# TheoBald200814/RGB-D-Instance-Segmentation

Hardware: AMD Instinct MI355X
Metric: NYUv2 640x480 RGB-D img/s (fwd+bwd) of the DGGM+E-DSAM hot path (higher is better)
Workload: dtype bf16

## Files before the change

### include/rgbd_hip.h

```cpp
#ifndef RGBD_HIP_H
#define RGBD_HIP_H

#include <stddef.h>
#include <stdint.h>

#ifdef __cplusplus
extern "C" {
#endif

#define RGBD_OK 0
#define RGBD_E_ARG (-1)
#define RGBD_E_SHAPE (-2)
#define RGBD_E_DTYPE (-3)

#define RGBD_F32 0
#define RGBD_BF16 1

#define RGBD_NBINS 512
#define RGBD_MAX_MODES 3

typedef struct rgbd_decomp_info {
  int32_t status;
  int32_t n_modes;
  int32_t n_masks;
// ... 64 lines not shown
                             const int* C_host, const int* h_host, const int* w_host, const float* grad,
                             const float* mask, long long pv_batch_stride, int B, int H, int W, void* ws,
                             void* stream);

int rgbd_nchw_to_nhwc(int dtype, const void* src, void* dst, int B, int C, int H, int W,
                      void* stream);
typedef struct rgbd_nhwc_job {
  const void* src;
  void* dst;
  int B, C, H, W;
} rgbd_nhwc_job;
int rgbd_nchw_to_nhwc_multi(int n, const rgbd_nhwc_job* jobs, void* stream);
typedef struct rgbd_nhwc_job_f32 {
  const void* src;
  void* dst;
  int B, C, H, W;
  int dst_dtype;
} rgbd_nhwc_job_f32;
int rgbd_nchw_to_nhwc_multi_f32(int n, const rgbd_nhwc_job_f32* jobs, void* stream);
long long rgbd_dsam_packed_elems(int dtype, int Cin, int Cout);
int rgbd_dsam_pack_weights(int dtype, const float* conv_w, const float* proj_w, int Cin,
                           int Cout, const uint32_t* code_mask, void* wfwd, void* wbwd, void* stream);
int rgbd_dsam_code_masks(int n, const uint8_t* const* codes_host, const long long* nbytes_host,
                         uint32_t* masks, void* stream);

size_t rgbd_dsam_conv_workspace_size(int dtype, int B, int Cin, int h, int w, int Cout);
int rgbd_dsam_fwd(int dtype, const void* x_nhwc, const uint8_t* code, const rgbd_decomp_info* info,
                  int B, int Cin, int h, int w, int Cout, const void* wfwd, const float* bias,
                  const void* residual, void* out_nchw, void* out_nhwc, void* ws, void* stream);
int rgbd_dsam_fwd_nhwc(int dtype, const void* x_nhwc, const uint8_t* code, const rgbd_decomp_info* info,
                       int B, int Cin, int h, int w, int Cout, const void* wfwd, const float* bias,
                       const void* residual_nhwc, void* out_nhwc, void* ws, void* stream);
int rgbd_dsam_fwd_nhwc_f32io(int dtype, const void* x_nhwc, const uint8_t* code, const rgbd_decomp_info* info,
                             int B, int Cin, int h, int w, int Cout, const void* wfwd, const float* bias,
                             const void* residual_nhwc, void* out_nhwc, void* ws, void* stream,
                             const float* residual_f32_nhwc, float* out_f32_nhwc);
int rgbd_dsam_bwd_data(int dtype, const void* gout_nhwc, const uint8_t* code, int B, int Cin, int h,
                       int w, int Cout, const void* wbwd, const void* gin_nchw, const void* gin_nhwc,
                       void* dx_nchw, void* dx_nhwc, void* ws, void* stream);
size_t rgbd_dsam_bwd_weight_workspace_size(int dtype, int B, int Cin, int h, int w, int Cout);
int rgbd_dsam_bwd_weight(int dtype, const void* gout_nchw, const void* gout_nhwc, const void* x_nhwc,
                         const uint8_t* code, const rgbd_decomp_info* info, int B, int Cin, int h,
                         int w, int Cout, float* dconv_w, float* dproj_w, float* dbias, void* ws,
                         void* stream);

enum { RGBD_LEG_FWD = 0, RGBD_LEG_DX = 1, RGBD_LEG_DW = 2 };
typedef struct rgbd_dsam_leg {
  int kind;
  const uint8_t* code;
  int B, Cin, h, w, Cout;
  void* plan;
} rgbd_dsam_leg;
size_t rgbd_dsam_plan_size(int kind, int B, int Cin, int h, int w, int Cout);
size_t rgbd_dsam_run_workspace_size(int kind, int B, int Cin, int h, int w, int Cout);
int rgbd_dsam_plan(int n, const rgbd_dsam_leg* legs, void* stream);
int rgbd_dsam_fwd_nhwc_planned(int dtype, const void* x_nhwc, const uint8_t* code,
                               const rgbd_decomp_info* info, int B, int Cin, int h, int w, int Cout,
                               const void* wfwd, const float* bias, const void* residual_nhwc,
                               void* out_nhwc, const void* plan, void* ws, void* stream);
int rgbd_dsam_fwd_nhwc_f32io_planned(int dtype, const void* x_nhwc, const uint8_t* code,
                                     const rgbd_decomp_info* info, int B, int Cin, int h, int w, int Cout,
                                     const void* wfwd, const float* bias, const void* residual_nhwc, void* out_nhwc,
                                     const void* plan, void* ws, void* stream, const float* residual_f32_nhwc,
                                     float* out_f32_nhwc);
int rgbd_dsam_bwd_data_planned(int dtype, const void* gout_nhwc, const uint8_t* code, int B, int Cin,
                               int h, int w, int Cout, const void* wbwd, const void* gin_nchw,
                               const void* gin_nhwc, void* dx_nchw, void* dx_nhwc, const void* plan,
                               void* ws, void* stream);
int rgbd_dsam_bwd_weight_planned(int dtype, const void* gout_nchw, const void* gout_nhwc,
                                 const void* x_nhwc, const uint8_t* code, const rgbd_decomp_info* info,
                                 int B, int Cin, int h, int w, int Cout, float* dconv_w, float* dproj_w,
                                 float* dbias, const void* plan, void* ws, void* stream);
typedef struct rgbd_dsam_dw_run {
  const void* gout_nhwc;
  const void* x_nhwc;
  const uint8_t* code;
  int B, Cin, h, w, Cout;
  float* dconv_w;
  float* dproj_w;
  float* dbias;
  const void* plan;
  void* ws;
} rgbd_dsam_dw_run;
int rgbd_dsam_bwd_weight_planned_multi(int n, const rgbd_dsam_dw_run* runs, const rgbd_decomp_info* info,
                                       void* stream);

int rgbd_adamw_multi(int n, float* const* params, const float* const* grads, float* const* exp_avg,
                     float* const* exp_avg_sq, const long long* numel, const float* step, double lr, double beta1,
                     double beta2, double eps, double weight_decay, void* stream);
int rgbd_adamw_multi_shadow(int n, float* const* params, const float* const* grads, float* const* exp_avg,
                            float* const* exp_avg_sq, void* const* shadows, const long long* numel,
                            const float* step, double lr, double beta1, double beta2, double eps,
                            double weight_decay, void* stream);

#define RGBD_RATIO_NW 24
#define RGBD_RATIO_NBN 6
size_t rgbd_ratio_packed_size(int dtype);
int rgbd_ratio_pack(int dtype, const float* const* weights_host, void* packed, void* stream);
size_t rgbd_ratio_workspace_size(int dtype, int B, int H, int W);
size_t rgbd_ratio_features_offset(int dtype, int B, int H, int W);
size_t rgbd_ratio_pooled_offset(int dtype, int B, int H, int W);
int rgbd_ratio_forward(int dtype, int training, float momentum, const float* depth3, long long batch_stride,
                       int B, int H, int W, const void* packed, float* const* bn_host, unsigned long long seed,
                       unsigned long long* seed_counter, float* ratio, void* ws, void* stream);
#define RGBD_RATIO_F_PHASE2 1
int rgbd_ratio_forward_ex(int dtype, int training, float momentum, const float* depth3, long long batch_stride,
// ... 116 lines not shown
```

### rgb-d-instance-segmentation_amd/_lib.py

```python
import ctypes
import os
from pathlib import Path

import numpy as np

LIB_PATH = Path(os.environ.get("RGBD_HIP_LIB", Path(__file__).resolve().parent / "librgbd_hip.so"))

RGBD_F32 = 0
RGBD_BF16 = 1
NBINS = 512

DECOMP_INFO_DTYPE = np.dtype([
    ("status", "<i4"), ("n_modes", "<i4"), ("n_masks", "<i4"), ("peak_bin", "<i4", 3),
    ("first_edge", "<f4"), ("last_edge", "<f4"), ("center", "<f4", 3),
    ("lo", "<f4", 3), ("hi", "<f4", 3), ("hist", "<i4", NBINS)])
assert DECOMP_INFO_DTYPE.itemsize == 2116

_P = ctypes.c_void_p
_I = ctypes.c_int
_LL = ctypes.c_longlong
_SZ = ctypes.c_size_t

SIGNATURES = {
    "rgbd_version": (ctypes.c_char_p, []),
    "rgbd_assemble_workspace_size": (_SZ, [_I]),
    "rgbd_assemble_pixel_values": (_I, [_P, _P, _I, _I, _I, _P, _P, _P]),
    "rgbd_instance_presence": (_I, [_P, _I, _I, _I, _P, _P]),
    "rgbd_instance_masks": (_I, [_P, _I, _I, _P, _P, _I, _P, _P]),
    "rgbd_pp_instance_workspace_size": (_SZ, [_I, _I]),
    "rgbd_pp_instance": (_I, [_P, _P, _I, _I, _I, _I, _I, _P, _P, ctypes.c_double, _P, _P, _P, _P, _P, _P]),
    "rgbd_pp_binary_maps": (_I, [_P, _I, _I, _I, _I, _I, _P, _P, _P]),
    "rgbd_pack_mask_bits": (_I, [_P, _I, _LL, _P, _P, _P]),
    "rgbd_mask_intersections": (_I, [_P, _I, _P, _I, _LL, _P, _P]),
    "rgbd_resize_workspace_size": (_SZ, [_I, _I, _I, _I, _I, _I]),
    "rgbd_resize_pil_bilinear": (_I, [_P, _I, _I, _I, _I, _I, _I, _P, _P, _P]),
    "rgbd_resize_pil_nearest": (_I, [_P, _I, _I, _I, _I, _I, _I, _P, _P, _P]),
    "rgbd_resize_cv2_linear": (_I, [_P, _I, _I, _I, _I, _I, _P, _P, _P]),
    "rgbd_edsam_decompose_workspace_size": (_SZ, [_I]),
    "rgbd_edsam_decompose": (_I, [_P, _LL, _I, _I, _I, _I, _P, _I, _P, _P, _P, _P, _P, _P]),
    "rgbd_edsam_decompose_masks": (_I, [_P, _LL, _I, _I, _I, _I, _P, _I, _P, _P, _P, _P, _P, _P, _P]),
    "rgbd_edsam_modes_workspace_size": (_SZ, [_I, _I, _I]),
    "rgbd_edsam_modes": (_I, [_P, _LL, _I, _I, _I, _I, _P, _P, _I, _P, _P]),
    "rgbd_edsam_codes": (_I, [_P, _I, _I, _I, _P, _I, _P, _P, _P, _P, _P, _P]),
    "rgbd_dggm_fuse_fwd": (_I, [_I, _P, _P, _P, _P, _LL, _I, _I, _I, _I, _I, _I, _P, _P, _P, _P]),
    "rgbd_dggm_fuse_bwd_workspace_size": (_SZ, [_I, _I, _I, _I]),
    "rgbd_dggm_fuse_bwd": (_I, [_I, _P, _P, _P, _LL, _I, _I, _I, _I, _I, _I, _P, _P, _P, _P, _P, _P]),
    "rgbd_dggm_fuse_fwd_multi": (_I, [_I, _I, _P, _P, _P, _P, _P, _P, _P, _P, _P, _P, _LL, _I, _I, _I, _P]),
    "rgbd_dggm_fuse_fwd_multi_mixed": (_I, [_I, _I, _P, _I, _P, _P, _P, _P, _P, _P, _P, _P, _P, _LL, _I, _I, _I,
                                            _P]),
    "rgbd_dggm_fuse_bwd_multi_workspace_size": (_SZ, [_I, _P, _P, _P, _I]),
    "rgbd_dggm_fuse_bwd_multi": (_I, [_I, _I, _P, _P, _P, _P, _P, _P, _P, _P, _P, _P, _LL, _I, _I, _I, _P, _P]),
    "rgbd_nchw_to_nhwc": (_I, [_I, _P, _P, _I, _I, _I, _I, _P]),
    "rgbd_nchw_to_nhwc_multi": (_I, [_I, _P, _P]),
    "rgbd_nchw_to_nhwc_multi_f32": (_I, [_I, _P, _P]),
    "rgbd_adamw_multi": (_I, [_I, _P, _P, _P, _P, _P, _P, ctypes.c_double, ctypes.c_double, ctypes.c_double,
                             ctypes.c_double, ctypes.c_double, _P]),
    "rgbd_adamw_multi_shadow": (_I, [_I, _P, _P, _P, _P, _P, _P, _P, ctypes.c_double, ctypes.c_double,
                                     ctypes.c_double, ctypes.c_double, ctypes.c_double, _P]),
    "rgbd_dsam_packed_elems": (_LL, [_I, _I, _I]),
    "rgbd_dsam_pack_weights": (_I, [_I, _P, _P, _I, _I, _P, _P, _P, _P]),
    "rgbd_dsam_code_masks": (_I, [_I, _P, _P, _P, _P]),
    "rgbd_dsam_conv_workspace_size": (_SZ, [_I, _I, _I, _I, _I, _I]),
    "rgbd_dsam_fwd": (_I, [_I, _P, _P, _P, _I, _I, _I, _I, _I, _P, _P, _P, _P, _P, _P, _P]),
    "rgbd_dsam_fwd_nhwc": (_I, [_I, _P, _P, _P, _I, _I, _I, _I, _I, _P, _P, _P, _P, _P, _P]),
    "rgbd_dsam_bwd_data": (_I, [_I, _P, _P, _I, _I, _I, _I, _I, _P, _P, _P, _P, _P, _P, _P]),
    "rgbd_dsam_bwd_weight_workspace_size": (_SZ, [_I, _I, _I, _I, _I, _I]),
    "rgbd_dsam_bwd_weight": (_I, [_I, _P, _P, _P, _P, _P, _I, _I, _I, _I, _I, _P, _P, _P, _P, _P]),
    "rgbd_dsam_plan_size": (_SZ, [_I, _I, _I, _I, _I, _I]),
    "rgbd_dsam_run_workspace_size": (_SZ, [_I, _I, _I, _I, _I, _I]),
    "rgbd_dsam_plan": (_I, [_I, _P, _P]),
    "rgbd_dsam_fwd_nhwc_planned": (_I, [_I, _P, _P, _P, _I, _I, _I, _I, _I, _P, _P, _P, _P, _P, _P, _P]),
    "rgbd_dsam_fwd_nhwc_f32io": (_I, [_I, _P, _P, _P, _I, _I, _I, _I, _I, _P, _P, _P, _P, _P, _P, _P, _P]),
    "rgbd_dsam_fwd_nhwc_f32io_planned": (_I, [_I, _P, _P, _P, _I, _I, _I, _I, _I, _P, _P, _P, _P, _P, _P, _P, _P,
                                              _P]),
    "rgbd_dsam_bwd_data_planned": (_I, [_I, _P, _P, _I, _I, _I, _I, _I, _P, _P, _P, _P, _P, _P, _P, _P]),
    "rgbd_dsam_bwd_weight_planned": (_I, [_I, _P, _P, _P, _P, _P, _I, _I, _I, _I, _I, _P, _P, _P, _P, _P, _P]),
    "rgbd_dsam_bwd_weight_planned_multi": (_I, [_I, _P, _P, _P]),
    "rgbd_point_sample": (_I, [_P, _I, _I, _I, _P, _I, _I, _P, _P]),
    "rgbd_point_sample_t": (_I, [_I, _P, _I, _I, _I, _P, _I, _I, _P, _P]),
    "rgbd_point_sample_sets": (_I, [_I, _P, _I, _I, _I, _P, _P, _I, _P, _P]),
    "rgbd_topk_rows_max_n": (_SZ, []),
    "rgbd_topk_rows": (_I, [_P, _I, _I, _I, _P, _P]),
    "rgbd_point_sample_bwd": (_I, [_P, _I, _I, _I, _P, _I, _I, _P, _P]),
    "rgbd_match_cost": (_I, [_P, _I, _I, _I, _P, _P, _P, _P, ctypes.c_float, ctypes.c_float, ctypes.c_float, _P, _P]),
    "rgbd_match_cost_probs": (_I, [_P, _I, _I, _I, _P, _P, _P, _I, _P, _P, ctypes.c_float, ctypes.c_float,
                                   ctypes.c_float, _P, _P]),
    "rgbd_point_losses": (_I, [_P, _P, _I, _I, _P, _P, _P, _P]),
    "rgbd_point_losses_bwd": (_I, [_P, _P, _I, _I, _P, _P, _P, _P, _P]),
    "rgbd_msda_fwd": (_I, [_I, _P, _I, _I, _P, _I, _I, _I, _I, _P, _P, _P, _P]),
    "rgbd_msda_bwd": (_I, [_I, _P, _I, _I, _P, _I, _I, _I, _I, _P, _P, _P, _P, _P, _P, _P]),
    "rgbd_level_memory_workspace_size": (_SZ, [_I, _I, _I]),
    "rgbd_level_memory_fwd": (_I, [_I, _P, _P, _I, _I, _I, _P, _P]),
    "rgbd_level_memory_bwd": (_I, [_I, _P, _I, _I, _I, _P, _P, _P, _P]),
    "rgbd_msda_locations": (_I, [_I, _P, _P, _P, _I, _I, _I, _I, _I, _P, _P]),
    "rgbd_msda_locations_bwd": (_I, [_I, _P, _P, _I, _I, _I, _I, _I, _P, _P]),
    "rgbd_lsa_lds_bytes": (_SZ, [_I, _I]),
    "rgbd_lsa_batch": (_I, [_I, _P, _P, _I, _I, _P, _P, _P, _P]),
    "rgbd_mask_logits": (_I, [_I, _P, _P, _I, _I, _I, _I, _I, _P, _P]),
    "rgbd_mask_attention": (_I, [_I, _P, _I, _I, _I, _I, _I, _I, _I, _P, _P]),
    "rgbd_masked_attn_fwd_workspace_size": (_SZ, [_I, _I, _I]),
    "rgbd_masked_attn_fwd": (_I, [_I, _P, _P, _P, _P, _I, _I, _I, _I, ctypes.c_float, _P, _P, _P, _P]),
    "rgbd_masked_attn_bwd_workspace_size": (_SZ, [_I, _I, _I]),
    "rgbd_masked_attn_bwd": (_I, [_I, _P, _P, _P, _P, _P, _P, _P, _I, _I, _I, _I, ctypes.c_float, _P, _P, _P, _P,
                                  _P]),
    "rgbd_gemm_workspace_size": (_SZ, [_I, _I, _I, _I]),
    "rgbd_gemm": (_I, [_I, _I, _I, _I, _I, _I, _P, _LL, _LL, _P, _LL, _LL, _P, _I, _P, _LL, _LL, _P, _LL, _LL, _I,
                       _I, _I, _P, _P]),
    "rgbd_im2col": (_I, [_I, _P, _I, _I, _I, _I, _I, _P, _P]),
    "rgbd_colsum_workspace_size": (_SZ, [_I, _I]),
    "rgbd_colsum": (_I, [_I, _P, _I, _I, _LL, _P, _P, _P]),
    "rgbd_layernorm_fwd": (_I, [_I, _P, _P, _P, _I, _I, ctypes.c_float, _I, _P, _P, _P, _P]),
    "rgbd_add_layernorm_fwd": (_I, [_I, _P, _I, _P, _P, _P, _I, _I, ctypes.c_float, ctypes.c_float, _I, _P, _P, _P,
                                    _P, _P, _P]),
    "rgbd_add_layernorm_bwd": (_I, [_I, _P, _I, _P, _P, _P, _P, _P, _I, _I, ctypes.c_float, _P, _P, _P, _P, _P,
                                    _P]),
    "rgbd_layernorm_bwd_workspace_size": (_SZ, [_I, _I]),
    "rgbd_layernorm_bwd": (_I, [_I, _P, _I, _P, _P, _P, _P, _I, _I, _P, _P, _P, _P, _P]),
    "rgbd_groupnorm_workspace_size": (_SZ, [_I, _I]),
    "rgbd_groupnorm_fwd": (_I, [_I, _P, _P, _P, _I, _I, _I, _I, ctypes.c_float, _I, _I, _P, _P, _P, _P]),
    "rgbd_groupnorm_bwd": (_I, [_I, _P, _I, _P, _P, _P, _P, _I, _I, _I, _I, _I, _P, _P, _P, _P, _P]),
    "rgbd_swin_window_attn": (_I, [_I, _P, _P, _P, _LL, _P, _P, _P, _P, _I, _I, _I, _I, _I, _I, ctypes.c_float, _P,
                                   _LL, _P]),
    "rgbd_timing_enable": (_I, [_I]),
# ... 62 lines not shown
```

### rgb-d-instance-segmentation_amd/csrc/dsam_conv.hip

```cpp
#include <cstdlib>

#include "mfma.hpp"
#include "timing.hpp"

using namespace rgbd;

namespace {

enum { MASK_NONE = 0, MASK_SRC = 1, MASK_DST = 2 };

struct ConvArgs {
  const void* x;
  const uint8_t* code;
  const void* w;
  int B, Hi, Wi, C;
  int Ho, Wo, N;
  int KH, KW, stride, pad;
  int nseg, mask_mode, transposed;
  const float* bias4;
  const rgbd_decomp_info* info;
  const void* residual;
  const void* residual_nhwc;
  void* out_nchw;
  void* out_nhwc;
// ... 1108 lines not shown
__device__ __forceinline__ bool ld_row(const ConvArgs& a, const LdGeom& G, int tile, int ml, int& b, int& i,
                                       int& j, int& org, uint32_t& rv, uint32_t& lo, uint32_t& hi) {
  int iq, jq;
  if (a.linear) {
    const int hw = G.Hc * G.Wc, m = tile * LD_BM + ml;
    b = m / hw;
    const int rem = m - b * hw;
    iq = rem / G.Wc;
    jq = rem - iq * G.Wc;
  } else {
    b = tile / (G.tiles_x * G.tiles_y);
    const int trem = tile - b * G.tiles_x * G.tiles_y;
    iq = (trem / G.tiles_x) * 8 + (ml >> 4);
    jq = (trem % G.tiles_x) * 16 + (ml & 15);
  }
  const bool mv = b < a.B && iq < G.Hc && jq < G.Wc;
  b = mv ? b : 0;
  i = mv ? iq : 0;
  j = mv ? jq : 0;
  rv = lo = hi = 0u;
  uint32_t cv[9];
  if (a.transposed) {
    const uint32_t rc = a.code[((long long)b * a.Ho + 2 * i + G.py) * a.Wo + 2 * j + G.px];
    org = mv ? (b * a.Hi + i) * a.Wi + j : 0;
#pragma unroll
    for (int t = 0; t < 9; ++t) {
      int ky, kx, dy, dx;
      ld_tap(a, G, t < G.ntap ? t : 0, ky, kx, dy, dx);
      if (mv && t < G.ntap && i + dy < a.Hi && j + dx < a.Wi) rv |= 1u << t;
      cv[t] = rc;
    }
  } else {
    org = mv ? (b * a.Hi + 2 * i - 1) * a.Wi + 2 * j - 1 : 0;
    int off[9];
#pragma unroll
    for (int t = 0; t < 9; ++t) {
      const int iy = 2 * i - 1 + t / 3, ix = 2 * j - 1 + t % 3;
      const bool inb = mv && iy >= 0 && iy < a.Hi && ix >= 0 && ix < a.Wi;
      if (inb) rv |= 1u << t;
      off[t] = inb ? org + (t / 3) * a.Wi + t % 3 : 0;
    }
#pragma unroll
    for (int t = 0; t < 9; ++t) cv[t] = a.code[off[t]];
  }
#pragma unroll
  for (int t = 0; t < 9; ++t)
    if ((rv >> t) & 1u) {
      const uint32_t c = cv[t] & 15u;
      if (t < 8) lo |= c << (4 * t); else hi |= c;
    }
  return mv;
}
__device__ __forceinline__ int ld_steps(const uint16_t* tm, int ntap, int ncg) {
  int s = 0;
  for (int t = 0; t < ntap; ++t) s += __popc((uint32_t)tm[t]) * ncg;
  return s;
}
__device__ __forceinline__ int ld_nchunks(int steps, int len) {
  const int n = (steps + len - 1) / len;
  return n < 1 ? 1 : (n > LD_CH ? LD_CH : n);
}

__device__ __forceinline__ void plan_tile(const ConvArgs& a, int cls, int tile, int ntn) {
  __shared__ uint32_t tm_s[9];
  const int ntiles0 = a.ntiles0, tid = threadIdx.x;
  const LdGeom G = ld_geom(a, cls);
  if (tile >= G.ntiles) return;
  if (tid < 9) tm_s[tid] = 0u;
  __syncthreads();
  int b, i, j, org;
  uint32_t rv, lo, hi;
  ld_row(a, G, tile, tid, b, i, j, org, rv, lo, hi);
  uint32_t tm[5] = {0u, 0u, 0u, 0u, 0u};
#pragma unroll
  for (int t = 0; t < 9; ++t)
    if ((rv >> t) & 1u) {
      const uint32_t c = (t < 8 ? lo >> (4 * t) : hi) & 15u;
      tm[t >> 1] |= (1u << c) << (16 * (t & 1));
    }
#pragma unroll
  for (int q = 0; q < 5; ++q)
#pragma unroll
    for (int o = 1; o < 64; o <<= 1) tm[q] |= (uint32_t)__shfl_xor((int)tm[q], o);
  if ((tid & 63) == 0)
#pragma unroll
    for (int t = 0; t < 9; ++t) {
      const uint32_t v = (tm[t >> 1] >> (16 * (t & 1))) & 0xffffu;
      if (v) atomicOr(&tm_s[t], v);
    }
  __syncthreads();
  if (tid < 16) a.tmasks[((long long)cls * ntiles0 + tile) * 16 + tid] = tid < 9 ? (uint16_t)tm_s[tid] : 0;
  if (cls == 0 && tile == 0 && tid < LD_ZERO_BYTES / 16)
    reinterpret_cast<uint4*>(const_cast<bf16_t*>(a.zero))[tid] = make_uint4(0u, 0u, 0u, 0u);
  for (int q = tid; q < ntn; q += 128) a.tickets[((long long)cls * ntiles0 + tile) * ntn + q] = 0;
  if (cls == 0 && tile == 0 && tid < ntn) a.work[tid] = 0;
}

constexpr int PLAN_MAXLEG = 8;
struct PlanLegs {
  ConvArgs a[PLAN_MAXLEG];
  int zb[PLAN_MAXLEG + 1];
  int ntn[PLAN_MAXLEG];
  int n;
};
__global__ __launch_bounds__(128) void k_dsam_plan(const PlanLegs L) {
  const int z = blockIdx.z;
  int leg = 0;
  while (leg + 1 < L.n && z >= L.zb[leg + 1]) ++leg;
  plan_tile(L.a[leg], z - L.zb[leg], blockIdx.x, L.ntn[leg]);
}

__device__ __forceinline__ void items_body(const ConvArgs& a) {
  __shared__ int wsum[16];
  __shared__ int base_s;
  const int ntiles0 = a.ntiles0, ncg = a.ncg;
  const int tid = threadIdx.x, lane = tid & 63, w = tid >> 6;
  const int nclass = a.transposed ? 4 : 1, total = nclass * ntiles0;
  if (tid == 0) base_s = 0;
  __syncthreads();
  for (int e0 = 0; e0 < total; e0 += 1024) {
    const int e = e0 + tid;
    int nc = 0;
    if (e < total) {
      const int ce = e / ntiles0, tile = e - ce * ntiles0;
      const int cls = a.transposed ? (0x0213 >> (4 * ce)) & 15 : ce;
      const LdGeom G = ld_geom(a, cls);
      if (tile < G.ntiles)
        nc = ld_nchunks(ld_steps(a.tmasks + ((long long)cls * ntiles0 + tile) * 16, G.ntap, ncg), a.chunk_len);
    }
    int x = nc;
#pragma unroll
    for (int o = 1; o < 64; o <<= 1) {
      const int y = __shfl_up(x, o);
      if (lane >= o) x += y;
    }
    if (lane == 63) wsum[w] = x;
    __syncthreads();
    int before = base_s;
    for (int q = 0; q < w; ++q) before += wsum[q];
    const int off = before + x - nc;
    if (e < total) {
      const int ce = e / ntiles0, tile = e - ce * ntiles0;
      const int cls = a.transposed ? (0x0213 >> (4 * ce)) & 15 : ce;
      for (int c = 0; c < nc; ++c) a.items[off + c] = cls | (c << 2) | (tile << 5);
    }
    __syncthreads();
    if (tid == 1023) base_s = off + nc;
    __syncthreads();
  }
  if (tid == 0) *a.nitems = base_s;
}
__global__ __launch_bounds__(1024) void k_dsam_items(const PlanLegs L) { items_body(L.a[blockIdx.x]); }

constexpr int LD_STAMP_ITEMS = 4;
__device__ __forceinline__ void ld_stamp(unsigned long long* st, int f) {
  if (!st) return;
  __builtin_amdgcn_sched_barrier(0);
  const unsigned long long t = __builtin_amdgcn_s_memtime();
  if (threadIdx.x == 0) st[f] = t;
  __builtin_amdgcn_sched_barrier(0);
}

template <int KC, int NODMA = 0, bool F32IO = false>
__device__ __forceinline__ void ld_item(const ConvArgs& a, int cls, int tile, int chunk, int ntile, int ntn,
                                        int* next_s, int nitems, unsigned long long* st = nullptr) {
  using Cfg = LdCfg<KC>;
  constexpr int S = Cfg::S;
  extern __shared__ __attribute__((aligned(1024))) char smem[];
  int4* rowtab = (int4*)(smem + Cfg::ROWTAB);
  int4* rowout = (int4*)(smem + Cfg::ROWOUT);
  float* bsum = (float*)(smem + Cfg::BSUM);
  const int tid = threadIdx.x, lane = tid & 63;
  const int wave = __builtin_amdgcn_readfirstlane(tid >> 6);
  const int r = lane & 15, g = lane >> 4;
  const int wm = wave & 1, wn = wave >> 1;
  const LdGeom G = ld_geom(a, cls);
  const int ncg = a.C / (32 * KC);
  const uint16_t* tmg = a.tmasks + ((long long)cls * a.ntiles0 + tile) * 16;
  uint32_t tmask[9];
  {
    const uint4 q0 = reinterpret_cast<const uint4*>(tmg)[0], q1 = reinterpret_cast<const uint4*>(tmg)[1];
    const uint32_t w[5] = {q0.x, q0.y, q0.z, q0.w, q1.x};
#pragma unroll
    for (int t = 0; t < 9; ++t) tmask[t] = t < G.ntap ? (w[t >> 1] >> (16 * (t & 1))) & 0xffffu : 0u;
  }
  int tb[10];
  tb[0] = 0;
#pragma unroll
  for (int t = 0; t < 9; ++t) tb[t + 1] = tb[t] + __popc(tmask[t]) * ncg;
  const int total = tb[9];
  const int nc = ld_nchunks(total, a.chunk_len);
  const int n0 = ntile * LD_BN;
  const bf16_t* xp = (const bf16_t*)a.x;
  const bf16_t* wp = (const bf16_t*)a.w;
  const uint32_t lds0 = (uint32_t)(uintptr_t)smem;
  for (int q = tid; q < G.ntap * ncg; q += 512) {
    const int t = q / ncg, cg = q - t * ncg;
    uint32_t msk = 0u;
    int e = 0;
#pragma unroll
    for (int u = 0; u < 9; ++u) {
      if (u == t) msk = tmask[u];
      if (u < t) e += __popc(tmask[u]) * ncg;
    }
    e += cg * __popc(msk);
    int* steptab = (int*)(smem + Cfg::STEPTAB);
    while (msk) {
      steptab[e++] = t | (cg << 4) | ((__ffs(msk) - 1) << 12);
      msk &= msk - 1u;
    }
  }
  if (tid < LD_BM) {
    int b, i, j, org;
    uint32_t rv, lo, hi;
    const bool mv = ld_row(a, G, tile, tid, b, i, j, org, rv, lo, hi);
    rowtab[tid] = make_int4(org, (int)rv, (int)lo, (int)hi);
    int obase = -1, opix = 0, nmk = 0;
    if (mv) {
      const int oy = a.transposed ? 2 * i + G.py : i, ox = a.transposed ? 2 * j + G.px : j;
      opix = (b * a.Ho + oy) * a.Wo + ox;
      obase = (b * a.N * a.Ho + oy) * a.Wo + ox;
      nmk = a.info ? a.info[b].n_masks : 0;
    }
    rowout[tid] = make_int4(obase, opix, nmk, 0);
  }
  __syncthreads();
  ld_stamp(st, 1);
  const int R = 16 * wave + (lane >> 2);
  int aorg, achk;
  uint32_t aval, alo, ahi;
  {
    const int4 e = rowtab[R];
    aorg = e.x;
    aval = (uint32_t)e.y;
    alo = (uint32_t)e.z;
    ahi = (uint32_t)e.w;
    achk = 8 * ((lane & 3) ^ lds_swz(R));
  }
  const int* steptab = (const int*)(smem + Cfg::STEPTAB);
  const bf16_t* zrow = a.zero + achk;
  const int s0 = (int)((long long)chunk * total / nc), s1 = (int)((long long)(chunk + 1) * total / nc);
  const int nst = s1 - s0;
  if (st && threadIdx.x == 0) st[6] = (unsigned long long)(nst | (nc << 16) | (chunk << 24));
  auto issue = [&](int slot, int s, bool inloop = false) {
// ... 303 lines not shown
        } else {
#pragma unroll
          for (int e = 0; e < 4; ++e) {
            const int4 re = rowout[ml + e];
            if (re.x >= 0) onchw[re.x + (long long)n * HoWo] = tv[e];
          }
        }
      }
    }
    }
    if (onhwc) {
      __syncthreads();
      const bool fused = !onchw;
      const bf16_t* rnhwc = (const bf16_t*)a.residual_nhwc;
      for (int it = tid; it < LD_BM * (HN / 8); it += 512) {
        const int ml = it % LD_BM, nl = (it / LD_BM) * 8, n = nh + nl;
        const int4 ro = rowout[ml];
        if (ro.x < 0 || n >= a.N) continue;
        float v[8];
#pragma unroll
        for (int e = 0; e < 8; ++e) v[e] = et[(nl + e) * LD_EPI_LD + ml];
        if (fused) {
#pragma unroll
          for (int e = 0; e < 8; ++e) v[e] += bsum[ro.z * LD_BN + half * HN + nl + e];
          if (rnhwc) {
            const uint4 u = *reinterpret_cast<const uint4*>(rnhwc + (long long)ro.y * a.N + n);
            const uint32_t uw[4] = {u.x, u.y, u.z, u.w};
#pragma unroll
            for (int e = 0; e < 4; ++e) {
              v[2 * e] = __uint_as_float(uw[e] << 16) + v[2 * e];
              v[2 * e + 1] = __uint_as_float(uw[e] & 0xffff0000u) + v[2 * e + 1];
            }
          }
        }
        *reinterpret_cast<uint4*>(onhwc + (long long)ro.y * a.N + n) =
            make_uint4(pack_bf16x2(v[0], v[1]), pack_bf16x2(v[2], v[3]), pack_bf16x2(v[4], v[5]), pack_bf16x2(v[6], v[7]));
      }
    }
  }
  ld_stamp(st, 5);
  publish();
}

template <int KC, bool STAMPS = false, int NODMA = 0, bool F32IO = false>
__global__ __launch_bounds__(512, 1) void k_dsam_lds(ConvArgs a) {
  using Cfg = LdCfg<KC>;
  extern __shared__ __attribute__((aligned(1024))) char smem[];
  if constexpr (NODMA != 0) {
    for (int e = threadIdx.x; e < Cfg::S * Cfg::STAGE / 16; e += 512)
      reinterpret_cast<uint4*>(smem)[e] = make_uint4(0u, 0u, 0u, 0u);
    __syncthreads();
  }
  int* next_s = (int*)(smem + Cfg::TMASK + 216);
  const int nitems = *a.nitems;
  const int ntile = blockIdx.y;
  {
    float* bsum = (float*)(smem + Cfg::BSUM);
    const int n0 = ntile * LD_BN;
    for (int e = threadIdx.x; e < 5 * LD_BN; e += 512) {
      const int k = e / LD_BN, nl = e - k * LD_BN, n = n0 + nl;
      float s = 0.f;
      if (a.bias4 && n < a.N)
        for (int sb = 0; sb < k; ++sb) s += a.bias4[sb * a.N + n];
      bsum[e] = s;
    }
  }
  if (threadIdx.x == 0) {
    const int it = __hip_atomic_fetch_add(a.work + ntile, 1, __ATOMIC_RELAXED, __HIP_MEMORY_SCOPE_AGENT);
    next_s[0] = it;
    next_s[1] = it < nitems ? a.items[it] : 0;
  }
  int done = 0;
  for (;;) {
    unsigned long long* st = nullptr;
    if constexpr (STAMPS) {
      if (done < LD_STAMP_ITEMS)
        st = a.stamps + ((long long)(blockIdx.x + blockIdx.y * gridDim.x) * LD_STAMP_ITEMS + done) * 8;
      ++done;
    }
    __syncthreads();
    const int it = next_s[0], v = next_s[1];
    if (it >= nitems) break;
    ld_stamp(st, 0);
    if (st && threadIdx.x == 0) st[7] = (unsigned long long)v;
    ld_item<KC, NODMA, F32IO>(a, v & 3, v >> 5, (v >> 2) & 7, ntile, gridDim.y, next_s, nitems, st);
  }
}


long long conv_mmax(const ConvArgs& a) {
  return a.transposed ? (long long)a.B * ((a.Ho + 1) / 2) * ((a.Wo + 1) / 2) : (long long)a.B * a.Ho * a.Wo;
}
int ld_kc(int C) { return C % 96 == 0 ? 3 : (C % 64 == 0 ? 2 : 1); }
int ld_linear(int Hc, int Wc) {
  const long long blk = (long long)((Hc + 7) / 8 * 8) * ((Wc + 15) / 16 * 16);
  return (long long)Hc * Wc * 100 < 85 * blk;
}
struct LdPlan {
  int ntiles0, ntn, kc, chunk_len, linear;
  size_t tmask_bytes, items_bytes, ticket_bytes, partial_bytes;
};
LdPlan ld_plan(const ConvArgs& a) {
  LdPlan p;
  const int Hc0 = a.transposed ? (a.Ho + 1) / 2 : a.Ho, Wc0 = a.transposed ? (a.Wo + 1) / 2 : a.Wo;
  const int nclass = a.transposed ? 4 : 1;
  p.linear = ld_linear(Hc0, Wc0);
  p.ntiles0 = p.linear ? (int)(((long long)a.B * Hc0 * Wc0 + LD_BM - 1) / LD_BM) : a.B * ((Hc0 + 7) / 8) * ((Wc0 + 15) / 16);
  p.ntn = ceil_div(a.N, LD_BN);
  p.kc = ld_kc(a.C);
  const int ntap = a.transposed ? 4 : 9;
  p.chunk_len = std::max(1, ntap * (a.C / (32 * p.kc)));
  p.tmask_bytes = align256((size_t)nclass * p.ntiles0 * 16 * sizeof(uint16_t));
  p.items_bytes = align256(((size_t)nclass * p.ntiles0 * LD_CH + 1) * sizeof(int));
  p.ticket_bytes = align256((size_t)(nclass * p.ntiles0 * p.ntn + 64) * sizeof(int)) + LD_ZERO_BYTES;
  p.partial_bytes = align256((size_t)nclass * p.ntiles0 * p.ntn * LD_CH * LD_BN * LD_BM * sizeof(float));
  return p;
}
size_t ld_plan_bytes(const LdPlan& p) { return p.tmask_bytes + p.items_bytes + p.ticket_bytes; }
size_t v2_partial_bytes(const ConvArgs& a) {
  const LdPlan p = ld_plan(a);
  return ld_plan_bytes(p) + p.partial_bytes;
}
ConvArgs conv_carve(const ConvArgs& a, const LdPlan& P, char* plan, float* partial) {
  ConvArgs b = a;
  const int nclass = a.transposed ? 4 : 1;
  b.tmasks = (uint16_t*)plan;
  b.items = (int*)(plan + P.tmask_bytes);
  b.nitems = b.items + (size_t)nclass * P.ntiles0 * LD_CH;
  b.tickets = (int*)(plan + P.tmask_bytes + P.items_bytes);
  b.work = b.tickets + (size_t)nclass * P.ntiles0 * P.ntn;
  b.zero = (const bf16_t*)(plan + ld_plan_bytes(P) - LD_ZERO_BYTES);
  b.partial = partial;
  b.ntiles0 = P.ntiles0;
  b.chunk_len = P.chunk_len;
  b.ncg = a.C / (32 * P.kc);
  b.linear = P.linear;
  return b;
}
bool conv_shape_ok(const ConvArgs& a, const LdPlan& P) {
  return a.C % 32 == 0 && a.N % 32 == 0 && (long long)a.B * a.Hi * a.Wi < (1ll << 31) && conv_mmax(a) < (1ll << 31) &&
         P.ntn <= 64 && 9 * 16 * (a.C / (32 * P.kc)) <= LD_MAXSTEP;
}
hipError_t plan_convs(int n, const ConvArgs* legs, hipStream_t s) {
  PlanLegs L = {};
  L.n = n;
  int z = 0, mt = 1;
  for (int i = 0; i < n; ++i) {
    L.a[i] = legs[i];
    L.zb[i] = z;
    L.ntn[i] = ceil_div(legs[i].N, LD_BN);
    z += legs[i].transposed ? 4 : 1;
    mt = std::max(mt, legs[i].ntiles0);
  }
  L.zb[n] = z;
  k_dsam_plan<<<dim3(mt, 1, z), 128, 0, s>>>(L);
  k_dsam_items<<<n, 1024, 0, s>>>(L);
  return hipGetLastError();
}

#ifdef RGBD_DIAG
unsigned long long* g_ld_stamps = nullptr;
int g_ld_stamp_cap = 0, g_ld_stamp_n = 0;
int g_ld_mode = 0;
template <int KC, int M>
hipError_t launch_ld_stamped(const ConvArgs& c, dim3 grid, hipStream_t s) {
  static const hipError_t sattr = hipFuncSetAttribute((const void*)k_dsam_lds<KC, true, M>,
// ... 576 lines not shown
  hipError_t e;
  if (n == 2 && fm[0] == fm[1]) {
    m.n = 2;
    e = launch_wg_fm(fm[0], m, s);
  } else {
    e = hipSuccess;
    for (int i = 0; i < n && e == hipSuccess; ++i) {
      WgMulti<1> one;
      one.a[0] = m.a[i];
      one.csum[0] = m.csum[i];
      one.n = 1;
      one.fold = 1;
      e = launch_wg_fm(fm[i], one, s);
    }
  }
  if (e != hipSuccess) return (int)e;
  if (n == 1)
    return wg_finish(m.a[0], nullptr, m.csum[0], info, runs[0].dconv_w, runs[0].dproj_w, runs[0].dbias, s, true);
  RGBD_REQUIRE(runs[0].Cin % FOLD_C == 0 && runs[1].Cin % FOLD_C == 0, RGBD_E_SHAPE);
  CombArgs c[2];
  for (int i = 0; i < 2; ++i)
    c[i] = comb_args(m.a[i], false, m.csum[i], info, runs[i].dconv_w, runs[i].dproj_w, runs[i].dbias);
  k_dsam_wgrad_fold<<<dim3(std::max(runs[0].Cin, runs[1].Cin) / FOLD_C, std::max(runs[0].Cout, runs[1].Cout), 2),
                      FOLD_T, 0, s>>>(c[0], c[1]);
  RGBD_CHECK_LAUNCH();
  return RGBD_OK;
}


static ConvArgs leg_conv_args(const rgbd_dsam_leg& g) {
  ConvArgs a = g.kind == RGBD_LEG_FWD ? fwd_args(g.B, g.Cin, g.h, g.w, g.Cout) : dx_args(g.B, g.Cin, g.h, g.w, g.Cout);
  a.code = g.code;
  return a;
}
static bool leg_ok(const rgbd_dsam_leg& g) {
  return (g.kind == RGBD_LEG_FWD || g.kind == RGBD_LEG_DX || g.kind == RGBD_LEG_DW) && g.B > 0 && g.h > 0 &&
         g.w > 0 && g.Cin > 0 && g.Cout > 0;
}
size_t rgbd_dsam_plan_size(int kind, int B, int Cin, int h, int w, int Cout) {
  const rgbd_dsam_leg g = {kind, nullptr, B, Cin, h, w, Cout, nullptr};
  if (!leg_ok(g)) return 0;
  if (kind == RGBD_LEG_DW) return wgrad_ws(RGBD_BF16, B, Cin, h, w, Cout).plan_total;
  return ld_plan_bytes(ld_plan(leg_conv_args(g)));
}
size_t rgbd_dsam_run_workspace_size(int kind, int B, int Cin, int h, int w, int Cout) {
  const rgbd_dsam_leg g = {kind, nullptr, B, Cin, h, w, Cout, nullptr};
  if (!leg_ok(g)) return 0;
  if (kind == RGBD_LEG_DW) {
    const WgradWs L = wgrad_ws(RGBD_BF16, B, Cin, h, w, Cout);
    return L.total - L.plan_total;
  }
  return std::max<size_t>(256, ld_plan(leg_conv_args(g)).partial_bytes);
}
#ifdef RGBD_DIAG
int rgbd_debug_dsam_stamps(void* buf, int launches) {
  RGBD_REQUIRE(buf ? launches > 0 : launches == 0, RGBD_E_ARG);
  g_ld_stamps = (unsigned long long*)buf;
  g_ld_stamp_cap = buf ? launches : 0;
  g_ld_stamp_n = 0;
  return RGBD_OK;
}
int rgbd_debug_dsam_mode(int mode) {
  RGBD_REQUIRE(mode == 0 || mode == 1 || mode == 2 || mode == 3 || mode == 7 || mode == 8 || mode == 15 || mode == 32 ||
                   mode == 64 || mode == 96,
               RGBD_E_ARG);
  g_ld_mode = mode;
  return RGBD_OK;
}
#endif

int rgbd_dsam_plan(int n, const rgbd_dsam_leg* legs, void* stream) {
  RGBD_REQUIRE(n > 0 && legs, RGBD_E_ARG);
  hipStream_t s = (hipStream_t)stream;
  ConvArgs conv[PLAN_MAXLEG];
  WgArgs wga[WG_MAXLEG];
  WgPlan wgp[WG_MAXLEG];
  int nconv = 0, nwg = 0;
  for (int i = 0; i < n; ++i) {
    const rgbd_dsam_leg& g = legs[i];
    RGBD_REQUIRE(leg_ok(g) && g.code && g.plan, RGBD_E_ARG);
    if (g.kind == RGBD_LEG_DW) {
      RGBD_REQUIRE(nwg < WG_MAXLEG, RGBD_E_ARG);
      const WgPlan P = wg_plan(g.B, g.Cin, g.h, g.w, g.Cout);
      RGBD_REQUIRE(wg_shape_ok(g.B, g.Cin, g.h, g.w, g.Cout, P), RGBD_E_SHAPE);
      const WgradWs L = wgrad_ws(RGBD_BF16, g.B, g.Cin, g.h, g.w, g.Cout);
      wgp[nwg] = P;
      wga[nwg++] = wg_args(L, P, (char*)g.plan, nullptr, nullptr, nullptr, g.code, g.B, g.Cin, g.h, g.w, g.Cout);
      continue;
    }
    RGBD_REQUIRE(nconv < PLAN_MAXLEG, RGBD_E_ARG);
    const ConvArgs a = leg_conv_args(g);
    const LdPlan P = ld_plan(a);
    RGBD_REQUIRE(conv_shape_ok(a, P), RGBD_E_SHAPE);
    conv[nconv++] = conv_carve(a, P, (char*)g.plan, nullptr);
  }
  if (nconv) {
    const hipError_t e = plan_convs(nconv, conv, s);
    if (e != hipSuccess) return (int)e;
  }
  if (nwg) wg_plan_launch(nwg, wga, wgp, s);
  RGBD_CHECK_LAUNCH();
  return RGBD_OK;
}

}
```

Measured before the change: 3086.

## Adapt DSAM chunk length to fill persistent grid and sort work items longest-first

The items planning kernel now picks a per-leg chunk length on device. When the tiles-times-N-tiles work count is below a persistent-block target, chunks are shortened so there are enough items to keep the grid busy; otherwise chunks are rounded evenly. Items are then bucketed by chunk length and ordered longest-first through a shared-memory counting sort, which should improve load balance in the persistent loop. The cost is extra planning work in a single block plus more split-K partial reductions when chunks get shorter.

```diff
diff --git a/include/rgbd_hip.h b/include/rgbd_hip.h
--- a/include/rgbd_hip.h
+++ b/include/rgbd_hip.h
@@ -140,6 +140,7 @@
   void* plan;
 } rgbd_dsam_leg;
 size_t rgbd_dsam_plan_size(int kind, int B, int Cin, int h, int w, int Cout);
+int rgbd_dsam_chunk_rule(const int* steps, int ntiles, int ntn, int dense, int* nchunks);
 size_t rgbd_dsam_run_workspace_size(int kind, int B, int Cin, int h, int w, int Cout);
 int rgbd_dsam_plan(int n, const rgbd_dsam_leg* legs, void* stream);
 int rgbd_dsam_fwd_nhwc_planned(int dtype, const void* x_nhwc, const uint8_t* code,
diff --git a/rgb-d-instance-segmentation_amd/_lib.py b/rgb-d-instance-segmentation_amd/_lib.py
--- a/rgb-d-instance-segmentation_amd/_lib.py
+++ b/rgb-d-instance-segmentation_amd/_lib.py
@@ -69,6 +69,7 @@
     "rgbd_dsam_plan_size": (_SZ, [_I, _I, _I, _I, _I, _I]),
     "rgbd_dsam_run_workspace_size": (_SZ, [_I, _I, _I, _I, _I, _I]),
     "rgbd_dsam_plan": (_I, [_I, _P, _P]),
+    "rgbd_dsam_chunk_rule": (_I, [_P, _I, _I, _I, _P]),
     "rgbd_dsam_fwd_nhwc_planned": (_I, [_I, _P, _P, _P, _I, _I, _I, _I, _I, _P, _P, _P, _P, _P, _P, _P]),
     "rgbd_dsam_fwd_nhwc_f32io": (_I, [_I, _P, _P, _P, _I, _I, _I, _I, _I, _P, _P, _P, _P, _P, _P, _P, _P]),
     "rgbd_dsam_fwd_nhwc_f32io_planned": (_I, [_I, _P, _P, _P, _I, _I, _I, _I, _I, _P, _P, _P, _P, _P, _P, _P, _P,
diff --git a/rgb-d-instance-segmentation_amd/csrc/dsam_conv.hip b/rgb-d-instance-segmentation_amd/csrc/dsam_conv.hip
--- a/rgb-d-instance-segmentation_amd/csrc/dsam_conv.hip
+++ b/rgb-d-instance-segmentation_amd/csrc/dsam_conv.hip
@@ -1184,13 +1184,46 @@
   return mv;
 }
 __device__ __forceinline__ int ld_steps(const uint16_t* tm, int ntap, int ncg) {
+  const uint4 q0 = reinterpret_cast<const uint4*>(tm)[0], q1 = reinterpret_cast<const uint4*>(tm)[1];
+  const uint32_t w[5] = {q0.x, q0.y, q0.z, q0.w, q1.x};
   int s = 0;
-  for (int t = 0; t < ntap; ++t) s += __popc((uint32_t)tm[t]) * ncg;
-  return s;
-}
-__device__ __forceinline__ int ld_nchunks(int steps, int len) {
-  const int n = (steps + len - 1) / len;
+#pragma unroll
+  for (int t = 0; t < 9; ++t) s += t < ntap ? __popc((w[t >> 1] >> (16 * (t & 1))) & 0xffffu) : 0;
+  return s * ncg;
+}
+constexpr int LD_PERS = 256;
+constexpr int LD_LMIN = 12;
+constexpr int LD_EVEN = 1 << 16;
+__host__ __device__ __forceinline__ int ld_div(int a, int b) {
+  return (int)(((unsigned)a & 0xffffu) / ((unsigned)b & 0xffffu));
+}
+__host__ __device__ __forceinline__ int ld_nchunks(int steps, int word) {
+  const int len = word & 0xffff;
+  const int n = (word & LD_EVEN) ? ld_div(2 * steps + len, 2 * len) : ld_div(steps + len - 1, len);
   return n < 1 ? 1 : (n > LD_CH ? LD_CH : n);
+}
+struct LdSumSelf {
+  __host__ __device__ int operator()(int v) const { return v; }
+};
+template <class Sum = LdSumSelf>
+__host__ __device__ inline int ld_chunk_rule(const int* steps, int ntiles, int ntn, int dense, int cfirst = 0,
+                                             int cstride = 1, int tfirst = 0, int tstride = 1, Sum sum = Sum()) {
+  auto items = [&](int word) {
+    int n = 0;
+    for (int t = tfirst; t < ntiles; t += tstride)
+      if (steps[t] >= 0) n += ld_nchunks(steps[t], word);
+    return sum(n) * ntn;
+  };
+  if (items(dense) >= LD_PERS) return dense | LD_EVEN;
+  for (int len = LD_LMIN + cfirst; len < dense; len += cstride)
+    if (items(len) <= LD_PERS) return len;
+  return dense;
+}
+__device__ __forceinline__ int* ld_chunk_word(const ConvArgs& a) { return a.nitems + 1; }
+constexpr int LD_NKEY = LD_MAXSTEP / 2 + (LD_MAXSTEP / 2) * LD_CH;
+__device__ __forceinline__ int ld_item_key(int len, int nc) {
+  len = len < 1 ? 1 : len;
+  return len > LD_MAXSTEP / 2 ? LD_MAXSTEP - len : LD_MAXSTEP / 2 + (LD_MAXSTEP / 2 - len) * LD_CH + (LD_CH - nc);
 }
 
 __device__ __forceinline__ void plan_tile(const ConvArgs& a, int cls, int tile, int ntn) {
@@ -1244,43 +1277,113 @@
 
 __device__ __forceinline__ void items_body(const ConvArgs& a) {
   __shared__ int wsum[16];
-  __shared__ int base_s;
+  __shared__ int word_s;
+  __shared__ int steps_s[1024];
+  __shared__ int cursor[LD_NKEY];
+  constexpr int KPT = LD_NKEY / 1024;
+  static_assert(KPT * 1024 == LD_NKEY, "buckets per thread");
   const int ntiles0 = a.ntiles0, ncg = a.ncg;
   const int tid = threadIdx.x, lane = tid & 63, w = tid >> 6;
   const int nclass = a.transposed ? 4 : 1, total = nclass * ntiles0;
-  if (tid == 0) base_s = 0;
+  const int ntn = (a.N + LD_BN - 1) / LD_BN;
+  auto load = [&](int e, int& cls, int& tile) {
+    const int ce = e / ntiles0;
+    tile = e - ce * ntiles0;
+    cls = a.transposed ? (0x0213 >> (4 * ce)) & 15 : ce;
+    const LdGeom G = ld_geom(a, cls);
+    return tile < G.ntiles ? ld_steps(a.tmasks + ((long long)cls * ntiles0 + tile) * 16, G.ntap, ncg) : -1;
+  };
+  auto entry = [&](int e, int& cls, int& tile) {
+    if (e >= 1024) return load(e, cls, tile);
+    const int ce = e / ntiles0;
+    tile = e - ce * ntiles0;
+    cls = a.transposed ? (0x0213 >> (4 * ce)) & 15 : ce;
+    return steps_s[e];
+  };
+  int ntl = 0;
+  for (int c = 0; c < nclass; ++c) ntl += ld_geom(a, c).ntiles;
+  for (int q = tid; q < LD_NKEY; q += 1024) cursor[q] = 0;
+  if (tid == 0) word_s = a.chunk_len | LD_EVEN;
+  {
+    int cls, tile;
+    steps_s[tid] = tid < total ? load(tid, cls, tile) : -1;
+  }
+  __syncthreads();
+  if ((long long)ntl * ntn < LD_PERS) {
+    auto wsum_i = [](int v) {
+#pragma unroll
+      for (int o = 1; o < 64; o <<= 1) v += __shfl_xor(v, o);
+      return v;
+    };
+    const int wd = ld_chunk_rule(steps_s, total, ntn, a.chunk_len, w, 16, lane, 64, wsum_i);
+    if (lane == 0) atomicMin(&word_s, wd);
+  }
+  __syncthreads();
+  if (tid == 0) *ld_chunk_word(a) = word_s;
+  __syncthreads();
+  const int word = *ld_chunk_word(a);
+  for (int e = tid; e < total; e += 1024) {
+    int cls, tile;
+    const int st = entry(e, cls, tile);
+    if (st >= 0) {
+      const int nc = ld_nchunks(st, word);
+      atomicAdd(&cursor[ld_item_key(ld_div(st + nc - 1, nc), nc)], nc);
+    }
+  }
+  __syncthreads();
+  {
+    int v[KPT], x = 0;
+#pragma unroll
+    for (int k = 0; k < KPT; ++k) x += v[k] = cursor[tid * KPT + k];
+    const int mine = x;
+#pragma unroll
+    for (int o = 1; o < 64; o <<= 1) {
+      const int y = __shfl_up(x, o);
+      if (lane >= o) x += y;
+    }
+    if (lane == 63) wsum[w] = x;
+    __syncthreads();
+    int off = x - mine;
+    for (int q = 0; q < w; ++q) off += wsum[q];
+#pragma unroll
+    for (int k = 0; k < KPT; ++k) {
+      cursor[tid * KPT + k] = off;
+      off += v[k];
+    }
+    if (tid == 1023) *a.nitems = off;
+  }
   __syncthreads();
   for (int e0 = 0; e0 < total; e0 += 1024) {
     const int e = e0 + tid;
-    int nc = 0;
+    int cls = 0, tile = 0, nc = 0, key = -1;
     if (e < total) {
-      const int ce = e / ntiles0, tile = e - ce * ntiles0;
-      const int cls = a.transposed ? (0x0213 >> (4 * ce)) & 15 : ce;
-      const LdGeom G = ld_geom(a, cls);
-      if (tile < G.ntiles)
-        nc = ld_nchunks(ld_steps(a.tmasks + ((long long)cls * ntiles0 + tile) * 16, G.ntap, ncg), a.chunk_len);
-    }
-    int x = nc;
-#pragma unroll
-    for (int o = 1; o < 64; o <<= 1) {
-      const int y = __shfl_up(x, o);
-      if (lane >= o) x += y;
-    }
-    if (lane == 63) wsum[w] = x;
-    __syncthreads();
-    int before = base_s;
-    for (int q = 0; q < w; ++q) before += wsum[q];
-    const int off = before + x - nc;
-    if (e < total) {
-      const int ce = e / ntiles0, tile = e - ce * ntiles0;
-      const int cls = a.transposed ? (0x0213 >> (4 * ce)) & 15 : ce;
-      for (int c = 0; c < nc; ++c) a.items[off + c] = cls | (c << 2) | (tile << 5);
-    }
-    __syncthreads();
-    if (tid == 1023) base_s = off + nc;
-    __syncthreads();
-  }
-  if (tid == 0) *a.nitems = base_s;
+      const int st = entry(e, cls, tile);
+      if (st >= 0) {
+        nc = ld_nchunks(st, word);
+        key = ld_item_key(ld_div(st + nc - 1, nc), nc);
+      }
+    }
+    int rank = 0, peers = 0;
+    for (unsigned long long todo = __ballot(key >= 0); todo;) {
+      const int k = __shfl(key, __ffsll((long long)todo) - 1);
+      const unsigned long long m = __ballot(key == k);
+      if (key == k) {
+        rank = __popcll(m & ((1ull << lane) - 1ull));
+        peers = __popcll(m);
+      }
+      todo &= ~m;
+    }
+    int off = 0;
+    const int nw = total - e0 < 1024 ? (total - e0 + 63) >> 6 : 16;
+    for (int ww = 0; ww < nw; ++ww) {
+      if (w == ww && key >= 0) {
+        off = cursor[key] + rank * nc;
+        if (rank == peers - 1) cursor[key] = off + nc;
+      }
+      __syncthreads();
+    }
+    for (int c = 0; c < nc; ++c) a.items[off + c] = cls | (c << 2) | (tile << 5);
+  }
 }
 __global__ __launch_bounds__(1024) void k_dsam_items(const PlanLegs L) { items_body(L.a[blockIdx.x]); }
 
@@ -1295,7 +1398,7 @@
 
 template <int KC, int NODMA = 0, bool F32IO = false>
 __device__ __forceinline__ void ld_item(const ConvArgs& a, int cls, int tile, int chunk, int ntile, int ntn,
-                                        int* next_s, int nitems, unsigned long long* st = nullptr) {
+                                        int* next_s, int nitems, int cword, unsigned long long* st = nullptr) {
   using Cfg = LdCfg<KC>;
   constexpr int S = Cfg::S;
   extern __shared__ __attribute__((aligned(1024))) char smem[];
@@ -1321,7 +1424,7 @@
 #pragma unroll
   for (int t = 0; t < 9; ++t) tb[t + 1] = tb[t] + __popc(tmask[t]) * ncg;
   const int total = tb[9];
-  const int nc = ld_nchunks(total, a.chunk_len);
+  const int nc = ld_nchunks(total, cword);
   const int n0 = ntile * LD_BN;
   const bf16_t* xp = (const bf16_t*)a.x;
   const bf16_t* wp = (const bf16_t*)a.w;
@@ -1731,7 +1834,7 @@
     __syncthreads();
   }
   int* next_s = (int*)(smem + Cfg::TMASK + 216);
-  const int nitems = *a.nitems;
+  const int nitems = *a.nitems, cword = *ld_chunk_word(a);
   const int ntile = blockIdx.y;
   {
     float* bsum = (float*)(smem + Cfg::BSUM);
@@ -1762,7 +1865,7 @@
     if (it >= nitems) break;
     ld_stamp(st, 0);
     if (st && threadIdx.x == 0) st[7] = (unsigned long long)v;
-    ld_item<KC, NODMA, F32IO>(a, v & 3, v >> 5, (v >> 2) & 7, ntile, gridDim.y, next_s, nitems, st);
+    ld_item<KC, NODMA, F32IO>(a, v & 3, v >> 5, (v >> 2) & 7, ntile, gridDim.y, next_s, nitems, cword, st);
   }
 }
 
@@ -1790,7 +1893,7 @@
   const int ntap = a.transposed ? 4 : 9;
   p.chunk_len = std::max(1, ntap * (a.C / (32 * p.kc)));
   p.tmask_bytes = align256((size_t)nclass * p.ntiles0 * 16 * sizeof(uint16_t));
-  p.items_bytes = align256(((size_t)nclass * p.ntiles0 * LD_CH + 1) * sizeof(int));
+  p.items_bytes = align256(((size_t)nclass * p.ntiles0 * LD_CH + 2) * sizeof(int));
   p.ticket_bytes = align256((size_t)(nclass * p.ntiles0 * p.ntn + 64) * sizeof(int)) + LD_ZERO_BYTES;
   p.partial_bytes = align256((size_t)nclass * p.ntiles0 * p.ntn * LD_CH * LD_BN * LD_BM * sizeof(float));
   return p;
@@ -2473,6 +2576,14 @@
   }
   return std::max<size_t>(256, ld_plan(leg_conv_args(g)).partial_bytes);
 }
+int rgbd_dsam_chunk_rule(const int* steps, int ntiles, int ntn, int dense, int* nchunks) {
+  RGBD_REQUIRE(steps && ntiles > 0 && ntn > 0 && dense > 0 && dense <= LD_MAXSTEP, RGBD_E_ARG);
+  for (int t = 0; t < ntiles; ++t) RGBD_REQUIRE(steps[t] <= LD_MAXSTEP, RGBD_E_ARG);
+  const int word = ld_chunk_rule(steps, ntiles, ntn, dense);
+  if (nchunks)
+    for (int t = 0; t < ntiles; ++t) nchunks[t] = steps[t] >= 0 ? ld_nchunks(steps[t], word) : 0;
+  return word & 0xffff;
+}
 #ifdef RGBD_DIAG
 int rgbd_debug_dsam_stamps(void* buf, int launches) {
   RGBD_REQUIRE(buf ? launches > 0 : launches == 0, RGBD_E_ARG);
```

Result: no change. 3107, median of 6 (+0.7%).
